# riddhiman13/predictive-multi-agent-framework

Measured on AMD Instinct MI355X. Metric: agent_rollouts_per_s, higher is better.
Workload: dtype f64; 1 GPU; C2: 64 agents x 200-step horizon, 32 sphere obstacles + repulsive sentinel, 1 population(s) per GPU (1 in the job) on 1 GPU(s), static obstacles, one pmaf_tick per step; agents=64, horizon=200, obstacles=32, populations_per_gpu=1, populations_total=1, parallelism=population-per-gpu x1 (same scene on every GPU), devices_visible=1, lanes_per_agent=64, rollout_blocks=64

## Files before the change

predictive-multi-agent-framework_amd/csrc/pmaf_rollout_w64.hpp:

```cpp
#pragma once
#include <type_traits>

#include "pmaf_device.hpp"

namespace pmaf {

template <int MATH>
__device__ __forceinline__ V3 attractor_velocity_error(V3 v, V3 goal_vec, const PopConst &C, double k_attr,
                                                       double k_damp) {
  V3 vel_des = (k_attr / k_damp) * goal_vec;
  double nd, rnd;
  Mth<MATH>::norm_rcp(vel_des, nd, rnd);
  double scale_lim = smin(1.0, Mth<MATH>::div_n(C.vel_max, nd, rnd));
  vel_des = vel_des * scale_lim;
  return vel_des - v;
}

template <int MATH>
__device__ __forceinline__ void finish_step_w64(V3 p, V3 &v, V3 verr, V3 F, double scale, const PopConst &C,
                                                double k_attr, double k_repel, double k_damp, V3 sent_pos,
                                                double sent_rad, double zsent_lt, V3 &new_pos,
                                                const bool sent_reachable = true) {
  if (sent_reachable) {
    V3 ro = sent_pos - p;
    V3 dist_vec = -ro;
    V3 repel = mk(0.0, 0.0, 0.0);
    if (sqn(dist_vec) < zsent_lt) {
      double d = norm(dist_vec) - (C.rad + sent_rad);
      d = smax(d, 1e-5);
      V3 otr = normalized(p - sent_pos);
      double t = 1.0 / d - 1.0 / C.shell;
      double dd = d * d;
      repel = ((k_repel * otr) * t) / dd;
    }
    V3 total = mk(0.0, 0.0, 0.0) + repel;
    F = F + total;
  }
  if (k_attr != 0.0) F = F + (scale * k_damp) * verr;
  V3 acc = F;
  if (C.mass != 1.0) acc = F / C.mass;
  const double az = sqn(acc);
  if (az >= C.zacc_gt) acc = acc * (13.0 / __builtin_sqrt(az));
  V3 half = ((0.5 * acc) * C.dt) * C.dt;
  new_pos = (p + half) + (v * C.dt);
  V3 nv = v + acc * C.dt;
  double vn, rvn;
  Mth<MATH>::norm_rcp(nv, vn, rvn);
  const double f = Mth<MATH>::div_n_pos(C.vel_max, vn, rvn);
  v = nv * ((vn > C.vel_max) ? f : 1.0);
}

__device__ __forceinline__ bool sentinel_reachable(V3 p, V3 sent_pos, V3 sent_vel, double zsent_lt, const PopConst &C,
                                                   int steps) {
  const double adt = fabs(C.dt);
  const double per_step = (6.5 * adt * adt + fabs(C.vel_max) * adt) + norm(sent_vel) * adt;
  const double reach = (double)steps * per_step * 1.001 + 1e-9;
  const double range = __builtin_sqrt(zsent_lt) * 1.001;
  const double d0 = norm(p - sent_pos);
  return !(d0 > range + reach);
}

__device__ __forceinline__ bool field_obstacles_at_rest(const double *src, int n_obs, int M, int lane, double dt) {
  bool rest = true;
  for (int i = lane; i < M; i += 64) {
    const unsigned long long bx = (unsigned long long)__double_as_longlong(src[3 * n_obs + i]),
                             by = (unsigned long long)__double_as_longlong(src[4 * n_obs + i]),
                             bz = (unsigned long long)__double_as_longlong(src[5 * n_obs + i]);
    const unsigned long long px = (unsigned long long)__double_as_longlong(src[i]),
                             py = (unsigned long long)__double_as_longlong(src[n_obs + i]),
                             pz = (unsigned long long)__double_as_longlong(src[2 * n_obs + i]);
    const unsigned long long neg0 = 0x8000000000000000ull;
    rest = rest && ((bx | by | bz) == 0ull) && (px != neg0) && (py != neg0) && (pz != neg0);
  }
  return !wave_any(!rest) && (dt >= 0.0) && (dt < __builtin_huge_val());
}

__device__ __forceinline__ V3 sentinel_repel(V3 p, const PopConst &C, double k_repel, V3 sent_pos, double sent_rad,
                                             double zsent_lt) {
  const V3 ro = sent_pos - p;
  const V3 dist_vec = -ro;
  V3 repel = mk(0.0, 0.0, 0.0);
  if (sqn(dist_vec) < zsent_lt) {
    double d = norm(dist_vec) - (C.rad + sent_rad);
    d = smax(d, 1e-5);
    const V3 otr = normalized(p - sent_pos);
    const double t = 1.0 / d - 1.0 / C.shell;
    const double dd = d * d;
    repel = ((k_repel * otr) * t) / dd;
  }
  return repel;
}

template <int MATH>
__device__ __forceinline__ V3 sentinel_repel_m(V3 p, const PopConst &C, double k_repel, V3 sent_pos, double sent_rad,
                                               double zsent_lt, double inv_shell) {
  typedef Mth<MATH> MT;
  const V3 ro = sent_pos - p;
  const V3 dist_vec = -ro;
  V3 repel = mk(0.0, 0.0, 0.0);
  const double z = sqn(dist_vec);
  if (z < zsent_lt) {
    const double s = MT::sqrt(z);
    double d = s - (C.rad + sent_rad);
    d = smax(d, 1e-5);
    const V3 pms = p - sent_pos;
    const double sd = (z > 0.0) ? s : 1.0;
    const V3 otr = MT::div3_n_pos(pms, sd, MT::rcp_for(sd));
    const double t = MT::div_pos(1.0, d) - inv_shell;
    const double dd = d * d;
    const V3 num = (k_repel * otr) * t;
    repel = MT::div3_n_pos(num, dd, MT::rcp_for(dd));
  }
  return repel;
}

__device__ __forceinline__ V3 sentinel_repel_live(V3 p, const PopConst &C, double k_repel, V3 sent_pos,
                                                  double sent_rad) {
  const V3 ro = sent_pos - p;
  const V3 dist_vec = -ro;
  V3 repel = mk(0.0, 0.0, 0.0);
  double d = norm(dist_vec) - (C.rad + sent_rad);
  d = smax(d, 1e-5);
  if (d < C.shell) {
    const V3 otr = normalized(p - sent_pos);
    const double t = 1.0 / d - 1.0 / C.shell;
    const double dd = d * d;
    repel = ((k_repel * otr) * t) / dd;
  }
  return repel;
}

__device__ __forceinline__ void wave_lds_fence() {
  __builtin_amdgcn_fence(__ATOMIC_RELEASE, "wavefront");
  __builtin_amdgcn_wave_barrier();
  __builtin_amdgcn_fence(__ATOMIC_ACQUIRE, "wavefront");
}

#ifdef PMAF_SECTION_TIMERS
struct SecTimers {
  unsigned long long last, acc[8], cnt[4];
  __device__ __forceinline__ void start() { for (int k = 0; k < 8; k++) acc[k] = 0; for (int k = 0; k < 4; k++) cnt[k] = 0; last = __builtin_amdgcn_s_memtime(); }
  __device__ __forceinline__ void mark(int k) { unsigned long long now = __builtin_amdgcn_s_memtime(); acc[k] += now - last; last = now; }
};
#define PMAF_SEC(ST, k) (ST).mark(k)
#define PMAF_CNT(ST, k, v) (ST).cnt[k] += (v)
#else
struct SecTimers {};
#define PMAF_SEC(ST, k)
#define PMAF_CNT(ST, k, v)
#endif

#define PMAF_RARE(c) __builtin_expect(!!(c), 0)

#ifndef PMAF_SUM_TAIL_PIN
#define PMAF_SUM_TAIL_PIN 0
#endif

typedef unsigned long long lmask;
#define PMAF_BAL(c) __builtin_amdgcn_ballot_w64(c)
#define PMAF_LANE(m) __builtin_amdgcn_inverse_ballot_w64(m)

template <int TILES>
struct LaneObstacles {
  V3 p[TILES], v[TILES];
  double r[TILES];
  double rx[TILES], ry[TILES], rz[TILES];
  double qx[TILES], qy[TILES], qz[TILES];
};

__device__ __forceinline__ int lane_rank(unsigned long long m) {
  return (int)__builtin_amdgcn_mbcnt_hi((unsigned)(m >> 32), __builtin_amdgcn_mbcnt_lo((unsigned)m, 0u));
}

__device__ __forceinline__ V3 readlane_v3(V3 a, int lane) {
  return mk(readlane_d(a.x, lane), readlane_d(a.y, lane), readlane_d(a.z, lane));
}

template <int TILES, int MATH>
__device__ __forceinline__ V3 closest_other_w64(lmask need_latch_m, int t, int lane, int M,
                                                const LaneObstacles<TILES> &O) {
  V3 cpos = mk(0.0, 0.0, 0.0);
  unsigned long long pend = need_latch_m;
  while (pend) {
    const int L = __ffsll((long long)pend) - 1;
    pend &= pend - 1;
    const int id = t * 64 + L;
    V3 own = mk(0.0, 0.0, 0.0);
#pragma unroll
    for (int u = 0; u < TILES; u++)
      if (u == t) own = readlane_v3(O.p[u], L);
    double bd = 100.0;
    int bj = 0x7fffffff;
#pragma unroll
    for (int u = 0; u < TILES; u++) {
      const int j = u * 64 + lane;
      const double d = Mth<MATH>::norm(own - O.p[u]);
      if (j < M && j != id && d < bd) { bd = d; bj = j; }
    }
    const double md = wave_min64(bd);
    const int mj = wave_min64_i((bj != 0x7fffffff && bd == md) ? bj : 0x7fffffff);
    const int c = (mj == 0x7fffffff) ? 0 : mj;
    V3 cp = mk(0.0, 0.0, 0.0);
#pragma unroll
    for (int u = 0; u < TILES; u++)
      if ((c >> 6) == u) cp = readlane_v3(O.p[u], c & 63);
    if (lane == L) cpos = cp;
  }
  return cpos;
}

template <int TILES>
__device__ __forceinline__ V3 closest_from_table_w64(const int32_t *cidx, int t, int lane, const LaneObstacles<TILES> &O) {
  const int c = cidx[t * 64 + lane];
  V3 cp = mk(0.0, 0.0, 0.0);
#pragma unroll
  for (int u = 0; u < TILES; u++) {
    const V3 q = mk(__shfl(O.p[u].x, c & 63), __shfl(O.p[u].y, c & 63), __shfl(O.p[u].z, c & 63));
    if ((c >> 6) == u) cp = q;
  }
  return cp;
}

template <int MATH>
__device__ __forceinline__ V3 cv_close_threshold(const V3 cur, const bool keep, V3 &quot) {
  typedef Mth<MATH> M;
  if constexpr (MATH == MATH_XACT) {
    const double z = sqn(cur);
    double y2;
    const double s = M::sqrt_seed(z, y2);
    quot = M::div3_n_pos(cur, s, M::rcp_seeded(s, y2));
    const bool tiny = (z < 0x1.79ca10c924223p-67) && !keep;
    return mk(tiny ? 0.0 : quot.x, tiny ? 0.0 : quot.y, tiny ? 1.0 : quot.z);
  } else {
    double s;
    M::template norm_unit<true>(cur, s, quot);
    const bool tiny = (s < 1e-10) && !keep;
    return mk(tiny ? 0.0 : quot.x, tiny ? 0.0 : quot.y, tiny ? 1.0 : quot.z);
  }
}

template <int TILES, int TYPE, int MATH, bool PRE = false, bool DPPSUM = false, class KT = ExpK, int NVL = -1, bool LONG = false>
__device__ __forceinline__ void circ_and_scale_w64(int lane, V3 p, V3 v, double zv, V3 goal, V3 g, double dg, V3 gn,
                                                   const PopConst &C, double k_circ,
                                                   int n_obs, double *rot_g, unsigned &known_bits,
                                                   LaneObstacles<TILES> &O, double *clist, double &lane_min,
                                                   V3 &F, double &scale, SecTimers &ST, const KT &EK,
                                                   const int rtype = 0,
                                                   const double s_pre = 0.0, const V3 ron_pre = V3{0.0, 0.0, 0.0},
                                                   const lmask gate_m = ~0ull, const int32_t *cidx = nullptr,
                                                   int *short_cap = nullptr) {
  static_assert(!LONG || (TILES == 1 && DPPSUM && TYPE != T_REAL), "the long loop belongs to the one-slot DPP sum of the rollout kernels");
  typedef Mth<MATH> MT;
  const int type = (TYPE == T_REAL) ? rtype : TYPE;
  constexpr int BATCH = 8;
  constexpr int SCRATCH = 64 * TILES + BATCH;
  constexpr int SUM_SCRATCH = (4 * TILES + 1) * 64;
  constexpr int MIN_CELL_BOUND = pmaf_list_area_doubles(TILES);
  (void)MIN_CELL_BOUND;
  (void)SCRATCH; (void)SUM_SCRATCH;
  const int M = n_obs - 1;
  double best_d = C.shell;
  double best_s = 0.0, best_gr = 0.0;
  int best_i = 0x7fffffff;
  lmask has_best_m = 0ull;
  V3 ron_t[TILES], rv_t[TILES];
  double d_t[TILES];
  lmask in_m[TILES];
  lmask any_in_m = 0ull;
#pragma unroll
  for (int t = 0; t < TILES; t++) {
    const int i = t * 64 + lane;
    const int left = M - t * 64;
    const lmask valid_m = gate_m & ((left >= 64) ? ~0ull : ((left <= 0) ? 0ull : ((1ull << left) - 1ull)));
    const V3 ro = O.p[t] - p;
    rv_t[t] = v - O.v[t];
    double s;
    if (PRE) { s = s_pre; ron_t[t] = ron_pre; }
    else MT::template norm_unit<true>(ro, s, ron_t[t]);
    const lmask skip_m = PMAF_BAL(dot(ron_t[t], gn) < -0.01) & PMAF_BAL(dot(ro, rv_t[t]) < -0.01);
    double d = s - (C.rad + O.r[t]);
    d = smax(d, 1e-5);
    d_t[t] = d;
    const lmask closer_m = valid_m & PMAF_BAL(d < best_d);
    has_best_m |= closer_m;
    const bool closer = PMAF_LANE(closer_m);
    if (TILES == 1) {
      if (closer) { best_d = d; best_i = i; }
      best_s = s; best_gr = dot(g, ro);
    } else {
      if (closer) { best_d = d; best_i = i; best_s = s; best_gr = dot(g, ro); }
    }
    const lmask live_m = valid_m & ~skip_m;
    if (PMAF_LANE(live_m & PMAF_BAL(d < lane_min))) lane_min = d;
    in_m[t] = live_m & PMAF_BAL(d < C.shell);
    any_in_m |= in_m[t];
  }
  PMAF_SEC(ST, 1);
  if (PMAF_RARE(any_in_m == 0ull)) return;
  PMAF_CNT(ST, 0, 1);
  constexpr int MIN_CELL = pmaf_list_area_doubles(TILES);
  unsigned long long *min_cell = reinterpret_cast<unsigned long long *>(clist + MIN_CELL);
  constexpr bool LDSMIN = DPPSUM;
  if (LDSMIN) {
    wave_lds_fence();
    *reinterpret_cast<double *>(min_cell) = C.shell;
    __hip_atomic_fetch_min(min_cell, (unsigned long long)__double_as_longlong(best_d), __ATOMIC_RELAXED,
                           __HIP_MEMORY_SCOPE_WORKGROUP);
  }

#pragma unroll
  for (int t = 0; t < TILES; t++) {
    const int i = t * 64 + lane;
    const lmask need_latch_m = in_m[t] & PMAF_BAL((known_bits & (1u << t)) == 0u);
    if (PMAF_RARE(need_latch_m != 0ull)) {
      V3 cpos = O.p[t];
      if (type == T_OBST || type == T_GOALOBST) {
        if (cidx) cpos = closest_from_table_w64<TILES>(cidx, t, lane, O);
        else cpos = closest_other_w64<TILES, MATH>(need_latch_m, t, lane, M, O);
      }
      if (PMAF_LANE(need_latch_m)) {
        V3 rot = calc_rot_vec_pre<MATH>(type, p, n_obs, O.p[t], cpos, mk(O.qx[t], O.qy[t], O.qz[t]), ron_t[t], g, dg, gn);
        rot_g[i] = rot.x; rot_g[n_obs + i] = rot.y; rot_g[2 * n_obs + i] = rot.z;
        O.rx[t] = rot.x; O.ry[t] = rot.y; O.rz[t] = rot.z;
        known_bits |= (1u << t);
      }
    }
  }
  PMAF_SEC(ST, 2);
  int count = 0;
  double m_mid = 0.0;
  if (LONG) {
    wave_lds_fence();
    clist[(16 << 2) + lane] = 0.0;
  }
  constexpr bool MIN_MID = TILES == 2;
#pragma unroll
  for (int t = 0; t < TILES; t++) {
    if (TILES > 2 && in_m[t] == 0ull) continue;
    const V3 rot = mk(O.rx[t], O.ry[t], O.rz[t]);
    const V3 rv = rv_t[t];
    constexpr bool NVR = (NVL >= 0) && PRE && TILES == 1 && TYPE != T_REAL;
    double zrv;
    V3 nv, cur;
    if constexpr (NVR) {
      zrv = zv;
      const bool rl = (lane == NVL);
      const V3 to_obs = ron_t[t];
      if constexpr (TYPE == T_VEL) {
        const V3 nvel = MT::template normalized<true>(rv);
        nv = nvel;
        V3 q;
        cur = cv_close_threshold<MATH>(nvel - to_obs * dot(nvel, to_obs), false, q);
      } else if constexpr (TYPE == T_GOAL) {
        V3 raw = g - to_obs * dot(to_obs, g);
        raw.x = rl ? v.x : raw.x; raw.y = rl ? v.y : raw.y; raw.z = rl ? v.z : raw.z;
        V3 q;
        cur = cv_close_threshold<MATH>(raw, rl, q);
        nv = readlane_v3(q, NVL);
      } else {
        V3 raw = cross(to_obs, rot);
        raw.x = rl ? v.x : raw.x; raw.y = rl ? v.y : raw.y; raw.z = rl ? v.z : raw.z;
        cur = MT::template normalized<true>(raw);
        nv = readlane_v3(cur, NVL);
      }
    } else {
      zrv = sqn(rv);
      double vn, rvn;
      MT::norm_rcp_zpos(zrv, vn, rvn);
      nv = MT::div3_n_pos(rv, vn, rvn);
      cur = current_vector<MATH, true>(type, rv, g, ron_t[t], rot);
    }
    if (LDSMIN && MIN_MID && t == TILES - 1) {
      wave_lds_fence();
      m_mid = __longlong_as_double((long long)__hip_atomic_load(min_cell, __ATOMIC_RELAXED, __HIP_MEMORY_SCOPE_WORKGROUP));
      __builtin_amdgcn_sched_barrier(0);
    }
    const V3 c = MT::div_pos(k_circ, d_t[t] * d_t[t]) * unit_triple<MATH>(nv, cur);
    const unsigned long long m = in_m[t] & PMAF_BAL(zrv != 0);
    const bool has_c = PMAF_LANE(m);
    if (DPPSUM) {
      const int sl = count + lane_rank(m);
      int li = ((sl >> 4) << 6) + (sl & 15);
      asm("" : "+v"(li));
      const int idx = has_c ? li : (SUM_SCRATCH + (lane >> 4) * 48 + (lane & 15));
      PMAF_BOUND(sl < 64 * TILES && idx + 32 < MIN_CELL_BOUND);
      clist[idx] = c.x; clist[idx + 16] = c.y; clist[idx + 32] = c.z;
    } else {
      const int slot = has_c ? (count + lane_rank(m)) : (SCRATCH + lane);
      PMAF_BOUND(slot * 4 + 2 < MIN_CELL_BOUND);
      double *e = clist + (size_t)slot * 4;
      e[0] = c.x; e[1] = c.y; e[2] = c.z;
    }
    count += __popcll(m);
  }
  if (DPPSUM) {
    if ((lane & 15) >= (count & 15)) clist[((count >> 4) << 6) + lane] = 0.0;
  } else {
    double *e = clist + (size_t)(count + (lane % BATCH)) * 4;
    e[0] = 0.0; e[1] = 0.0; e[2] = 0.0;
  }
  PMAF_CNT(ST, 1, count);
  double e_first = 0.0, e_second = 0.0;
  if (DPPSUM) {
    wave_lds_fence();
    e_first = clist[lane];
    if (TILES == 1) e_second = clist[(16 << 2) + lane];
  }

  double sc;
  {
    double m;
    if (LDSMIN && MIN_MID) {
      m = m_mid;
    } else if (LDSMIN) {
      wave_lds_fence();
      m = __longlong_as_double((long long)__hip_atomic_load(min_cell, __ATOMIC_RELAXED, __HIP_MEMORY_SCOPE_WORKGROUP));
    } else {
      m = wave_min64(best_d);
    }
    const lmask cand_m = has_best_m & PMAF_BAL(best_d == m);
    int bi;
    if (TILES == 1) {
      bi = cand_m ? (__ffsll((long long)cand_m) - 1) : 0x7fffffff;
    } else {
      bi = 0x7fffffff;
#pragma unroll
      for (int t = TILES - 1; t >= 0; t--) {
        const lmask ct = cand_m & PMAF_BAL((best_i >> 6) == t);
        bi = ct ? (t * 64 + __ffsll((long long)ct) - 1) : bi;
      }
    }
    const bool stall = (dot(g, v) <= 0.0) && (zv < C.zv09_lt) && (dg > 0.15);
    double w1;
    if (TILES >= 2) {
      typename std::remove_const<KT>::type EKs = EK;
      double m_in = m;
      const ExpHead H = exp_head(EKs, m_in);
      w1 = 1 - portable_exp_nonpos_staged(-MT::div_pos(MT::sqrt_pos(m_in), C.shell), EKs, H);
    }
    ExpPend EP;
    if (TILES == 1) EP = portable_exp_nonpos_begin(-MT::div_pos(MT::sqrt_pos(m), C.shell), EK);
    const int bl = bi & 63;
    const double sb = readlane_d(best_s, bl), gr = readlane_d(best_gr, bl);
    double w2 = 1 - MT::div(gr, dg * sb);
    w2 = w2 * w2;
    if (TILES == 1) w1 = 1 - portable_exp_nonpos_end(EP);
    const double w = w1 * w2;
    sc = (bi == 0x7fffffff) ? 1.0 : (stall ? 0.0 : w);
  }

  if (DPPSUM) {
  {
    double acc = 0.0;
    if (TILES >= 2) {
    double one = 1.0;
    asm volatile("" : "+v"(one));
    double e = e_first;
    int c16 = 0;
    {
      double en = clist[(16 << 2) + lane];
      asm volatile("s_nop 1" : "+v"(e));
#define PMAF_FM1(K) asm("v_fmac_f64_dpp %0, %1, %2 row_newbcast:" #K " row_mask:0xf bank_mask:0xf" : "+v"(acc) : "v"(e), "v"(one));
      PMAF_FM1(0) PMAF_FM1(1) PMAF_FM1(2) PMAF_FM1(3) PMAF_FM1(4) PMAF_FM1(5) PMAF_FM1(6) PMAF_FM1(7)
      PMAF_FM1(8) PMAF_FM1(9) PMAF_FM1(10) PMAF_FM1(11) PMAF_FM1(12) PMAF_FM1(13) PMAF_FM1(14) PMAF_FM1(15)
#undef PMAF_FM1
      asm volatile("s_nop 0" : "+v"(acc));
      e = en;
      c16 = 16;
      asm volatile("" : : "v"(sc));
    }
    for (; c16 < count; c16 += 16) {
      const double en = clist[((c16 + 16) << 2) + lane];
#define PMAF_FM(K) "v_fmac_f64_dpp %0, %1, %2 row_newbcast:" #K " row_mask:0xf bank_mask:0xf\n\t"
      asm volatile("s_nop 4\n\t"
                   PMAF_FM(0) PMAF_FM(1) PMAF_FM(2) PMAF_FM(3) PMAF_FM(4) PMAF_FM(5) PMAF_FM(6) PMAF_FM(7)
                   PMAF_FM(8) PMAF_FM(9) PMAF_FM(10) PMAF_FM(11) PMAF_FM(12) PMAF_FM(13) PMAF_FM(14) PMAF_FM(15)
                   "s_nop 1"
                   : "+v"(acc) : "v"(e), "v"(one));
#undef PMAF_FM
      e = en;
    }
    } else {
      double one = 1.0;
      asm volatile("" : "+v"(one));
      {
        double e = e_first;
        asm volatile("s_nop 1" : "+v"(e));
#define PMAF_FM1(K) asm("v_fmac_f64_dpp %0, %1, %2 row_newbcast:" #K " row_mask:0xf bank_mask:0xf" : "+v"(acc) : "v"(e), "v"(one));
        PMAF_FM1(0) PMAF_FM1(1) PMAF_FM1(2) PMAF_FM1(3) PMAF_FM1(4) PMAF_FM1(5) PMAF_FM1(6) PMAF_FM1(7)
        PMAF_FM1(8) PMAF_FM1(9) PMAF_FM1(10) PMAF_FM1(11) PMAF_FM1(12) PMAF_FM1(13) PMAF_FM1(14) PMAF_FM1(15)
#undef PMAF_FM1
      }
      if constexpr (LONG) {
        double e2 = e_second;
        asm("s_nop 1\n\tv_fmac_f64_dpp %0, %1, %2 row_newbcast:0 row_mask:0xf bank_mask:0xf" : "+v"(acc) : "v"(e2), "v"(one));
#define PMAF_FM1(K) asm("v_fmac_f64_dpp %0, %1, %2 row_newbcast:" #K " row_mask:0xf bank_mask:0xf" : "+v"(acc) : "v"(e2), "v"(one));
        PMAF_FM1(1) PMAF_FM1(2) PMAF_FM1(3) PMAF_FM1(4) PMAF_FM1(5) PMAF_FM1(6) PMAF_FM1(7)
        PMAF_FM1(8) PMAF_FM1(9) PMAF_FM1(10) PMAF_FM1(11) PMAF_FM1(12) PMAF_FM1(13) PMAF_FM1(14) PMAF_FM1(15)
#undef PMAF_FM1
        asm volatile("s_nop 0" : "+v"(acc));
        if (PMAF_SUM_TAIL_PIN) asm volatile("" : : "v"(sc), "v"(acc));
        if (PMAF_RARE(count > 32)) {
          double e = clist[(32 << 2) + lane];
          for (int c16 = 32; c16 < count; c16 += 16) {
            const double en = clist[((c16 + 16) << 2) + lane];
#define PMAF_FM(K) "v_fmac_f64_dpp %0, %1, %2 row_newbcast:" #K " row_mask:0xf bank_mask:0xf\n\t"
            asm volatile("s_nop 4\n\t"
                         PMAF_FM(0) PMAF_FM(1) PMAF_FM(2) PMAF_FM(3) PMAF_FM(4) PMAF_FM(5) PMAF_FM(6) PMAF_FM(7)
                         PMAF_FM(8) PMAF_FM(9) PMAF_FM(10) PMAF_FM(11) PMAF_FM(12) PMAF_FM(13) PMAF_FM(14) PMAF_FM(15)
                         "s_nop 1"
                         : "+v"(acc) : "v"(e), "v"(one));
#undef PMAF_FM
            e = en;
          }
        }
      } else {
      if (PMAF_SUM_TAIL_PIN) asm volatile("" : : "v"(sc), "v"(acc));
      double e = e_second;
      for (int c16 = 16; PMAF_RARE(c16 < count); c16 += 16) {
        const double en = clist[((c16 + 16) << 2) + lane];
#define PMAF_FM(K) "v_fmac_f64_dpp %0, %1, %2 row_newbcast:" #K " row_mask:0xf bank_mask:0xf\n\t"
        asm volatile("s_nop 4\n\t"
                     PMAF_FM(0) PMAF_FM(1) PMAF_FM(2) PMAF_FM(3) PMAF_FM(4) PMAF_FM(5) PMAF_FM(6) PMAF_FM(7)
                     PMAF_FM(8) PMAF_FM(9) PMAF_FM(10) PMAF_FM(11) PMAF_FM(12) PMAF_FM(13) PMAF_FM(14) PMAF_FM(15)
                     "s_nop 1"
                     : "+v"(acc) : "v"(e), "v"(one));
#undef PMAF_FM
        e = en;
        if (short_cap) asm volatile("s_mov_b32 %0, 0" : "=s"(*short_cap));
      }
      }
    }
    F = mk(readlane_d(acc, 0), readlane_d(acc, 16), readlane_d(acc, 32));
  }
  wave_lds_fence();
  } else {
  wave_lds_fence();
  if (TILES == 1 || lane == 0) {
  for (int k = 0;;) {
    double ex[BATCH], ey[BATCH], ez[BATCH];
#pragma unroll
    for (int j = 0; j < BATCH; j++) {
      const double *e = clist + (size_t)(k + j) * 4;
      ex[j] = e[0]; ey[j] = e[1]; ez[j] = e[2];
    }
#pragma unroll
    for (int j = 0; j < BATCH; j++) { F.x = F.x + ex[j]; F.y = F.y + ey[j]; F.z = F.z + ez[j]; }
    k += BATCH;
    if (k >= count) break;
  }
  }
  if (TILES > 1) F = readlane_v3(F, 0);
  wave_lds_fence();
  }
  PMAF_SEC(ST, 3);
  scale = (sqn(F) >= C.zf_gt) ? sc : scale;
  PMAF_SEC(ST, 4);
}

__device__ __forceinline__ double ld_agent(const double *p) {
  return __hip_atomic_load(p, __ATOMIC_RELAXED, __HIP_MEMORY_SCOPE_AGENT);
}
template <int MATH>
__device__ __forceinline__ void path_cost_terms_w64(int lane, const double *path, int n, const double *ws,
                                                    double k_workspace, double *list, double &cost_ws,
                                                    double &path_len) {
  __builtin_amdgcn_fence(__ATOMIC_RELEASE, "agent");
  __builtin_amdgcn_fence(__ATOMIC_ACQUIRE, "agent");
  cost_ws = 0.0;
  path_len = 0.0;
  V3 q_n = mk(0.0, 0.0, 0.0), qp_n = mk(0.0, 0.0, 0.0);
  auto fetch = [&](int base, V3 &q, V3 &qp) __attribute__((always_inline)) {
    const int k = base + lane;
    const bool valid = k < n;
    const bool has_seg = valid && (k > 0);
    const int kk = valid ? k : 0, kp = has_seg ? (k - 1) : 0;
    q = mk(ld_agent(path + kk * 3), ld_agent(path + kk * 3 + 1), ld_agent(path + kk * 3 + 2));
    qp = mk(ld_agent(path + kp * 3), ld_agent(path + kp * 3 + 1), ld_agent(path + kp * 3 + 2));
  };
  fetch(0, q_n, qp_n);
  for (int base = 0; base < n; base += 64) {
    const int k = base + lane;
    const bool valid = k < n;
    const bool has_seg = valid && (k > 0);
    const V3 q = q_n, qp = qp_n;
    if (base + 64 < n) fetch(base + 64, q_n, qp_n);
    const double seg = Mth<MATH>::norm(q - qp);
    list[lane] = has_seg ? seg : 0.0;
    wave_lds_fence();
#pragma unroll 8
    for (int j = 0; j < 64; j++) path_len += list[j];
    wave_lds_fence();
    const bool out = valid && ((q.x > ws[0]) | (q.x < ws[1]) | (q.y > ws[2]) | (q.y < ws[3]) | (q.z > ws[4]) | (q.z < ws[5]));
    unsigned long long m = wave_ballot(out);
    while (m) {
      const int L = __ffsll((long long)m) - 1;
      m &= m - 1;
      ws_cost_add(cost_ws, readlane_v3(q, L), ws, k_workspace);
    }
  }
}

}
```

predictive-multi-agent-framework_amd/csrc/pmaf_rollout_w64_body.hpp:

```cpp
#pragma once
#include <hip/hip_runtime.h>
#include <hip/hip_ext.h>

#include "pmaf_types.hpp"
#include "pmaf_device.hpp"
#include "pmaf_rollout_w64.hpp"
#include "pmaf_rollout_grp.hpp"

using namespace pmaf;

#define PMAF_W64_EACH_TYPE(type, BODY) \
  switch (type) { \
    case T_GOAL: BODY(T_GOAL); break; \
    case T_OBST: BODY(T_OBST); break; \
    case T_GOALOBST: BODY(T_GOALOBST); break; \
    case T_VEL: BODY(T_VEL); break; \
    case T_RANDOM: BODY(T_RANDOM); break; \
    case T_HAD: BODY(T_HAD); break; \
    default: break; \
  }

__device__ __forceinline__ bool track_reachable(int lane, V3 p0, const double *trk, int n_pts, double zsent_lt,
                                                const PopConst &C, int steps) {
  const double adt = fabs(C.dt);
  const double per_step = 6.5 * adt * adt + fabs(C.vel_max) * adt;
  const double reach = (double)steps * per_step * 1.001 + 1e-9;
  const double range = __builtin_sqrt(zsent_lt) * 1.001;
  bool any = false;
  for (int j = lane; j < n_pts; j += 64) {
    const V3 y = mk(trk[3 * j], trk[3 * j + 1], trk[3 * j + 2]);
    any = any || !(norm(p0 - y) > range + reach);
  }
  return wave_any(any);
}

__device__ __forceinline__ double *w64_exp_lds() {
  __shared__ double s_expk[EXPK_N];
  return s_expk;
}
template <int TILES>
__device__ __forceinline__ auto w64_exp_consts(int lane) {
  if constexpr (TILES >= 2) {
    double *tab = w64_exp_lds();
    exp_consts_to_lds(tab, lane);
    wave_lds_fence();
    return exp_consts_from_lds(tab);
  } else {
    return exp_consts_in_vgprs();
  }
}
template <int TILES, int TYPE, int MATH, int SENT = 2, bool DPPSUM = false, bool PLAIN = false, bool STATICV = false, bool SLICE = false,
          bool TRACK = false, bool FTRACK = false>
__device__ __forceinline__ void rollout_w64_body(const DevView &D, const CostParams &CP, const int lane,
                                                 const int pop, const int a, const double *trk = nullptr,
                                                 const int trk_len = 0, const double *ftrk = nullptr,
                                                 const int ftrk_len = 0, const int ftrk_first = 0) {
  static_assert(!TRACK || (TILES == 1 && SENT != 2), "the repulsive track rides in lane 60 of the one-slot kernel");
  static_assert(!FTRACK || (TILES == 1 && SENT != 2 && !STATICV && TRACK), "the obstacle tracks ride in lanes 0 .. M-1 of the one-slot kernel");
  extern __shared__ double smem[];
  const unsigned long long t_begin = wall_clock64();
  const int n_obs = D.n_obs;
  const int M = n_obs - 1;
  PopConst C = D.C;
  { double *f = reinterpret_cast<double *>(&C);
    for (int i = 0; i < (int)(sizeof(PopConst) / sizeof(double)); i++) asm volatile("" : "+v"(f[i])); }
  const auto EK = w64_exp_consts<TILES>(lane);
  const size_t pa = (size_t)pop * D.N + a;
  const double *src = D.obs_start + (size_t)pop * 7 * n_obs;
  const int32_t *ks = D.known_start + (size_t)pop * n_obs;
  double *rot_g = D.rot + pa * 3 * n_obs;
  const double *rnd_g = D.rnd + pa * 3 * n_obs;

  LaneObstacles<TILES> O;
  unsigned known_bits = 0u;
  constexpr bool USES_CLOSEST = TILES >= 2 && (TYPE == T_OBST || TYPE == T_GOALOBST);
#pragma unroll
  for (int t = 0; t < TILES; t++) {
    int i = t * 64 + lane;
    bool valid = i < M;
    int ii = valid ? i : 0;
    O.p[t] = mk(src[ii], src[n_obs + ii], src[2 * n_obs + ii]);
    O.v[t] = mk(src[3 * n_obs + ii], src[4 * n_obs + ii], src[5 * n_obs + ii]);
    O.r[t] = src[6 * n_obs + ii];
    O.rx[t] = rot_g[ii]; O.ry[t] = rot_g[n_obs + ii]; O.rz[t] = rot_g[2 * n_obs + ii];
    if (TYPE == T_RANDOM) { O.qx[t] = rnd_g[ii]; O.qy[t] = rnd_g[n_obs + ii]; O.qz[t] = rnd_g[2 * n_obs + ii]; }
    else { O.qx[t] = 0.0; O.qy[t] = 0.0; O.qz[t] = 0.0; }
    if (valid && ks[ii]) known_bits |= (1u << t);
  }
  V3 sent_p = mk(src[M], src[n_obs + M], src[2 * n_obs + M]);
  const V3 sent_v = mk(src[3 * n_obs + M], src[4 * n_obs + M], src[5 * n_obs + M]);
  const double sent_r = src[6 * n_obs + M];
  typedef const __attribute__((address_space(1))) double *gptr;
  gptr trk_v = (gptr)trk;
  const int trk_last = (trk_len > 0) ? (trk_len - 1) : 0;
  const lmask trk_m = (TRACK && SENT == 1 && trk_len > 0) ? (1ull << 60) : 0ull;
  if (TRACK && SENT == 1) {
    asm volatile("" : "+v"(trk_v));
    if (trk_len > 0) sent_p = mk(trk_v[0], trk_v[1], trk_v[2]);
  }
  gptr ftrk_v = (gptr)ftrk + lane;
  const int ftrk_last = (ftrk_len > 0) ? (ftrk_len - 1) : 0;
  const int ftrk_at = (ftrk_first < ftrk_last) ? ftrk_first : ftrk_last;
  const lmask ftrk_m = (FTRACK && ftrk_len > 0) ? ((1ull << M) - 1ull) : 0ull;
  if (FTRACK) {
    asm volatile("" : "+v"(ftrk_v));
    const gptr fp = ftrk_v + (size_t)ftrk_at * 384;
    const bool fl = PMAF_LANE(ftrk_m);
    O.p[0].x = fl ? fp[0] : O.p[0].x; O.p[0].y = fl ? fp[64] : O.p[0].y; O.p[0].z = fl ? fp[128] : O.p[0].z;
    O.v[0].x = fl ? fp[192] : O.v[0].x; O.v[0].y = fl ? fp[256] : O.v[0].y; O.v[0].z = fl ? fp[320] : O.v[0].z;
  }

  V3 goal = mk(D.goal[pop * 3], D.goal[pop * 3 + 1], D.goal[pop * 3 + 2]);
  V3 init_pos = mk(D.agent_init_pos[pop * 3], D.agent_init_pos[pop * 3 + 1], D.agent_init_pos[pop * 3 + 2]);
  asm volatile("" : "+v"(goal.x), "+v"(goal.y), "+v"(goal.z), "+v"(init_pos.x), "+v"(init_pos.y), "+v"(init_pos.z));
  V3 p = mk(D.start_pos[pop * 3], D.start_pos[pop * 3 + 1], D.start_pos[pop * 3 + 2]);
  V3 v = mk(D.start_vel[pop * 3], D.start_vel[pop * 3 + 1], D.start_vel[pop * 3 + 2]);
  double k_attr = D.k_attr[pa], k_circ = D.k_circ[pa], k_repel = D.k_repel[pa], k_damp = D.k_damp[pa];
  asm volatile("" : "+v"(k_attr), "+v"(k_circ), "+v"(k_repel), "+v"(k_damp));
  double *path = D.paths + pa * (size_t)D.cap * 3;

  int clist_off = 7 * n_obs + (n_obs + 1) / 2;
  clist_off += clist_off & 1;
  double *clist = smem + clist_off;

  double lane_min = C.shell;
  int n = 1;
  bool ran = false;
  if (lane == 0) { path[0] = p.x; path[1] = p.y; path[2] = p.z; }

  typedef Mth<MATH> MT;
  V3 g = goal - p;
  double dg = MT::norm(g);
  double zv = sqn(v);
  double z_init = sqn(p - init_pos);
  V3 gn = (dg > 0.0) ? MT::div3(g, dg) : g;
  constexpr bool PRE = (TILES == 1);
  double s_pre = 0.0;
  V3 ron_pre = mk(0.0, 0.0, 0.0);
  double lane_scale = (lane == 61) ? (k_attr / k_damp) : 1.0;
  asm volatile("" : "+v"(lane_scale));
  if (PRE) {
    const double nz = (C.dt < 0.0) ? 0.0 : -0.0;
    if (lane == 63 || lane == 61) { O.p[0] = goal; O.v[0] = mk(nz, nz, nz); }
    if (SENT == 1 && lane == 60) { O.p[0] = sent_p; O.v[0] = sent_v; }
    MT::norm_unit(O.p[0] - p, s_pre, ron_pre);
  }
  constexpr bool SRIDE = PRE && SENT == 1;
  V3 verr = attractor_velocity_error<MATH>(v, g, C, k_attr, k_damp);
  const double zsent_lt = D.zsent_lt[pop];
  const bool sent_reachable = (SENT == 2) ? sentinel_reachable(p, sent_p, sent_v, zsent_lt, C, D.cap) : (SENT == 1);
  bool moving = false;
#pragma unroll
  for (int t = 0; t < TILES; t++) moving = moving || !(O.v[t].x == 0.0 && O.v[t].y == 0.0 && O.v[t].z == 0.0);
  moving = wave_any(moving);
  bool advance = true;
  const int32_t *cidx = nullptr;
  if (USES_CLOSEST) {
    if (!moving && D.closest_ok[pop] == 1) {
      int32_t *s_cidx = reinterpret_cast<int32_t *>(smem);
      const int32_t *ci = D.closest_idx + (size_t)pop * n_obs;
#pragma unroll
      for (int t = 0; t < TILES; t++) {
        const int i = t * 64 + lane;
        if (i < M) s_cidx[i] = ci[i];
      }
      wave_lds_fence();
      cidx = s_cidx;
    }
  }
  V3 repel = mk(0.0, 0.0, 0.0);
  const double inv_shell = (SENT == 0) ? 0.0 : 1.0 / C.shell;
  if (sent_reachable) repel = sentinel_repel_m<MATH>(p, C, k_repel, sent_p, sent_r, zsent_lt, inv_shell);
  SecTimers ST;
#ifdef PMAF_SECTION_TIMERS
  ST.start();
#endif
  const bool younger = SLICE && ((((unsigned)blockIdx.y * gridDim.x + blockIdx.x) / (unsigned)D.n_simds) & 1u) != 0u;
  const unsigned slice_log2 = (unsigned)D.prio_slice_log2, younger_of_8 = (unsigned)D.prio_younger_of_8;
  if constexpr (TILES == 1 && DPPSUM) {
    int short_cap = D.cap;
    while ((dg > 0.1) && (n < short_cap)) {
#define PMAF_STEP_LONG false
#define PMAF_STEP_FLAG , &short_cap
#include "pmaf_rollout_w64_step.hpp"
#undef PMAF_STEP_LONG
    }
    while ((dg > 0.1) && (n < D.cap)) {
#define PMAF_STEP_LONG true
#include "pmaf_rollout_w64_step.hpp"
#undef PMAF_STEP_LONG
#undef PMAF_STEP_FLAG
    }
  } else {
    while ((dg > 0.1) && (n < D.cap)) {
#define PMAF_STEP_LONG false
#define PMAF_STEP_FLAG
#include "pmaf_rollout_w64_step.hpp"
#undef PMAF_STEP_LONG
#undef PMAF_STEP_FLAG
    }
  }
  if (SLICE) __builtin_amdgcn_s_setprio(0);
#ifdef PMAF_SECTION_TIMERS
  if (lane == 0 && pop == 0 && a < 7)
    printf("agent %d type %d steps %d | verr+gate %llu sweep %llu scale %llu circ %llu sum %llu (skip) %llu finish %llu tail %llu | "
           "in-shell steps %llu terms %llu\n", a, TYPE, n - 1, ST.acc[0], ST.acc[1], ST.acc[2], ST.acc[3], ST.acc[4],
           ST.acc[5], ST.acc[6], ST.acc[7], ST.cnt[0], ST.cnt[1]);
#endif

  double cost_ws, path_len;
#ifdef PMAF_SECTION_TIMERS
  const unsigned long long t_loop_end = wall_clock64();
#endif
  path_cost_terms_w64<MATH>(lane, path, n, CP.ws, CP.k_workspace, clist, cost_ws, path_len);
#ifdef PMAF_SECTION_TIMERS
  if (lane == 0 && pop == 0 && a < 7)
    printf("agent %d: loop %llu0 ns, path-cost pass %llu0 ns (%d points)\n", a, t_loop_end - t_begin, wall_clock64() - t_loop_end, n);
#endif

  const double min_obs = wave_min64(lane_min);
  int32_t *ko = D.known_out + pa * n_obs;
#pragma unroll
  for (int t = 0; t < TILES; t++) {
    int i = t * 64 + lane;
    if (i < M) ko[i] = (int32_t)((known_bits >> t) & 1u);
  }
  if (lane == 0) {
    ko[M] = ks[M];
    D.n_points[pa] = n;
    D.agent_vel[pa * 3] = v.x; D.agent_vel[pa * 3 + 1] = v.y; D.agent_vel[pa * 3 + 2] = v.z;
    D.min_obs[pa] = min_obs;
    D.cost_ws[pa] = cost_ws;
    D.path_len[pa] = path_len;
    D.goal_dist[pa] = dg;
    if (ran) D.reached[pa] = dg < 0.100001;
    atomicAdd(D.step_counter, (unsigned long long)(n - 1));
    D.pred_ticks[pa] = wall_clock64() - t_begin;
  }
}

template <int TILES, int MATH, bool DPPSUM, bool PLAIN, bool SLICE>
__device__ __forceinline__ void rollout_w64_dispatch(const DevView &D, const CostParams &CP) {
  const int lane = threadIdx.x;
  const int pop = blockIdx.y;
  const int a = blockIdx.x;
  if (TILES == 1) {
    const int n_obs = D.n_obs, M = n_obs - 1;
    const double *src = D.obs_start + (size_t)pop * 7 * n_obs;
    const V3 sp = mk(src[M], src[n_obs + M], src[2 * n_obs + M]);
    const V3 sv = mk(src[3 * n_obs + M], src[4 * n_obs + M], src[5 * n_obs + M]);
    const V3 p0 = mk(D.start_pos[pop * 3], D.start_pos[pop * 3 + 1], D.start_pos[pop * 3 + 2]);
    const PopConst C0 = D.C;
    const bool reach = sentinel_reachable(p0, sp, sv, D.zsent_lt[pop], C0, D.cap);
    const bool st = field_obstacles_at_rest(src, n_obs, M, lane, C0.dt) && (M <= 59 || !reach);
#define PMAF_BODY(T) \
    if (st) { \
      if (!reach) rollout_w64_body<TILES, T, MATH, 0, DPPSUM, PLAIN, true, SLICE>(D, CP, lane, pop, a); \
      else rollout_w64_body<TILES, T, MATH, 1, DPPSUM, PLAIN, true, SLICE>(D, CP, lane, pop, a); \
    } else if (!reach) rollout_w64_body<TILES, T, MATH, 0, DPPSUM, PLAIN, false, SLICE>(D, CP, lane, pop, a); \
    else rollout_w64_body<TILES, T, MATH, 1, DPPSUM, PLAIN, false, SLICE>(D, CP, lane, pop, a)
    PMAF_W64_EACH_TYPE(D.types[a], PMAF_BODY)
#undef PMAF_BODY
    return;
  }
#define PMAF_BODY(T) rollout_w64_body<TILES, T, MATH, 2, DPPSUM, PLAIN>(D, CP, lane, pop, a)
  PMAF_W64_EACH_TYPE(D.types[a], PMAF_BODY)
#undef PMAF_BODY
}
```

Before: 280,700 rollouts/s.

## Batch path-cost pass over four chunks with DPP broadcast-FMA path-length sum

Restructures the post-rollout path-cost pass to fetch four 64-point chunks of the path at once, which raises memory-level parallelism over the single-chunk prefetch it replaces. The serial 64-element LDS sum per chunk is replaced with inline-asm v_fmac_f64_dpp row_newbcast instructions that accumulate 16 values per issue. The wave-min reduction of the obstacle distance is moved inside the function so it can overlap with the outstanding loads. This adds hand-written asm with manual s_nop hazard padding, which is arch-specific and may change the floating-point summation order.

```diff
diff --git a/predictive-multi-agent-framework_amd/csrc/pmaf_rollout_w64.hpp b/predictive-multi-agent-framework_amd/csrc/pmaf_rollout_w64.hpp
--- a/predictive-multi-agent-framework_amd/csrc/pmaf_rollout_w64.hpp
+++ b/predictive-multi-agent-framework_amd/csrc/pmaf_rollout_w64.hpp
@@ -561,44 +561,90 @@
 __device__ __forceinline__ double ld_agent(const double *p) {
   return __hip_atomic_load(p, __ATOMIC_RELAXED, __HIP_MEMORY_SCOPE_AGENT);
 }
+#define PMAF_FM(K) "v_fmac_f64_dpp %0, %1, %2 row_newbcast:" #K " row_mask:0xf bank_mask:0xf\n\t"
+__device__ __forceinline__ void path_sum_chunk(double &acc, double e, double one) {
+  asm volatile("s_nop 4\n\t"
+               PMAF_FM(0) PMAF_FM(1) PMAF_FM(2) PMAF_FM(3) PMAF_FM(4) PMAF_FM(5) PMAF_FM(6) PMAF_FM(7)
+               PMAF_FM(8) PMAF_FM(9) PMAF_FM(10) PMAF_FM(11) PMAF_FM(12) PMAF_FM(13) PMAF_FM(14) PMAF_FM(15)
+               "s_nop 1"
+               : "+v"(acc) : "v"(e), "v"(one));
+}
+#undef PMAF_FM
 template <int MATH>
 __device__ __forceinline__ void path_cost_terms_w64(int lane, const double *path, int n, const double *ws,
                                                     double k_workspace, double *list, double &cost_ws,
-                                                    double &path_len) {
+                                                    double &path_len, const double *lane_min = nullptr,
+                                                    double *wave_min = nullptr) {
   __builtin_amdgcn_fence(__ATOMIC_RELEASE, "agent");
   __builtin_amdgcn_fence(__ATOMIC_ACQUIRE, "agent");
   cost_ws = 0.0;
-  path_len = 0.0;
-  V3 q_n = mk(0.0, 0.0, 0.0), qp_n = mk(0.0, 0.0, 0.0);
-  auto fetch = [&](int base, V3 &q, V3 &qp) __attribute__((always_inline)) {
-    const int k = base + lane;
-    const bool valid = k < n;
-    const bool has_seg = valid && (k > 0);
-    const int kk = valid ? k : 0, kp = has_seg ? (k - 1) : 0;
-    q = mk(ld_agent(path + kk * 3), ld_agent(path + kk * 3 + 1), ld_agent(path + kk * 3 + 2));
-    qp = mk(ld_agent(path + kp * 3), ld_agent(path + kp * 3 + 1), ld_agent(path + kp * 3 + 2));
+  constexpr int NB = 4;
+  V3 q[NB], qp[NB];
+  auto fetch = [&](int base) __attribute__((always_inline)) {
+#pragma unroll
+    for (int b = 0; b < NB; b++) {
+      const int k = base + 64 * b + lane;
+      const bool valid = k < n;
+      const bool has_seg = valid && (k > 0);
+      const int kk = valid ? k : 0, kp = has_seg ? (k - 1) : 0;
+      q[b] = mk(ld_agent(path + kk * 3), ld_agent(path + kk * 3 + 1), ld_agent(path + kk * 3 + 2));
+      qp[b] = mk(ld_agent(path + kp * 3), ld_agent(path + kp * 3 + 1), ld_agent(path + kp * 3 + 2));
+    }
   };
-  fetch(0, q_n, qp_n);
-  for (int base = 0; base < n; base += 64) {
-    const int k = base + lane;
-    const bool valid = k < n;
-    const bool has_seg = valid && (k > 0);
-    const V3 q = q_n, qp = qp_n;
-    if (base + 64 < n) fetch(base + 64, q_n, qp_n);
-    const double seg = Mth<MATH>::norm(q - qp);
-    list[lane] = has_seg ? seg : 0.0;
-    wave_lds_fence();
-#pragma unroll 8
-    for (int j = 0; j < 64; j++) path_len += list[j];
-    wave_lds_fence();
-    const bool out = valid && ((q.x > ws[0]) | (q.x < ws[1]) | (q.y > ws[2]) | (q.y < ws[3]) | (q.z > ws[4]) | (q.z < ws[5]));
-    unsigned long long m = wave_ballot(out);
-    while (m) {
-      const int L = __ffsll((long long)m) - 1;
-      m &= m - 1;
-      ws_cost_add(cost_ws, readlane_v3(q, L), ws, k_workspace);
-    }
-  }
-}
-
-}
+  fetch(0);
+  if (lane_min) *wave_min = wave_min64(*lane_min);
+  double acc = 0.0, one = 1.0;
+  asm volatile("" : "+v"(one));
+  const int col = lane & 15;
+  for (int base = 0;;) {
+    double seg[NB], e[NB][4];
+#pragma unroll
+    for (int b = 0; b < NB; b++) seg[b] = Mth<MATH>::norm(q[b] - qp[b]);
+#pragma unroll
+    for (int b = 0; b < NB; b++) {
+      int lane_w = lane;
+      asm volatile("" : "+v"(lane_w));
+      const int k = base + 64 * b + lane_w;
+      const bool has_seg = (k < n) && (k > 0);
+      list[lane] = has_seg ? seg[b] : 0.0;
+      wave_lds_fence();
+#pragma unroll
+      for (int j = 0; j < 4; j++) e[b][j] = list[(j << 4) + col];
+      wave_lds_fence();
+    }
+#pragma unroll
+    for (int b = 0; b < NB; b++) {
+      const int nb = n - base - 64 * b;
+      if (nb > 0) {
+        path_sum_chunk(acc, e[b][0], one);
+        if (nb > 16) {
+          path_sum_chunk(acc, e[b][1], one);
+          if (nb > 32) {
+            path_sum_chunk(acc, e[b][2], one);
+            if (nb > 48) path_sum_chunk(acc, e[b][3], one);
+          }
+        }
+      }
+    }
+#pragma unroll
+    for (int b = 0; b < NB; b++) {
+      int lane_o = lane;
+      asm volatile("" : "+v"(lane_o));
+      const bool valid = base + 64 * b + lane_o < n;
+      const V3 qb = q[b];
+      const bool out = valid && ((qb.x > ws[0]) | (qb.x < ws[1]) | (qb.y > ws[2]) | (qb.y < ws[3]) | (qb.z > ws[4]) | (qb.z < ws[5]));
+      unsigned long long m = wave_ballot(out);
+      while (m) {
+        const int L = __ffsll((long long)m) - 1;
+        m &= m - 1;
+        ws_cost_add(cost_ws, readlane_v3(qb, L), ws, k_workspace);
+      }
+    }
+    base += 64 * NB;
+    if (base >= n) break;
+    fetch(base);
+  }
+  path_len = acc;
+}
+
+}
diff --git a/predictive-multi-agent-framework_amd/csrc/pmaf_rollout_w64_body.hpp b/predictive-multi-agent-framework_amd/csrc/pmaf_rollout_w64_body.hpp
--- a/predictive-multi-agent-framework_amd/csrc/pmaf_rollout_w64_body.hpp
+++ b/predictive-multi-agent-framework_amd/csrc/pmaf_rollout_w64_body.hpp
@@ -212,13 +212,13 @@
 #ifdef PMAF_SECTION_TIMERS
   const unsigned long long t_loop_end = wall_clock64();
 #endif
-  path_cost_terms_w64<MATH>(lane, path, n, CP.ws, CP.k_workspace, clist, cost_ws, path_len);
+  double min_obs;
+  path_cost_terms_w64<MATH>(lane, path, n, CP.ws, CP.k_workspace, clist, cost_ws, path_len, &lane_min, &min_obs);
 #ifdef PMAF_SECTION_TIMERS
   if (lane == 0 && pop == 0 && a < 7)
     printf("agent %d: loop %llu0 ns, path-cost pass %llu0 ns (%d points)\n", a, t_loop_end - t_begin, wall_clock64() - t_loop_end, n);
 #endif
 
-  const double min_obs = wave_min64(lane_min);
   int32_t *ko = D.known_out + pa * n_obs;
 #pragma unroll
   for (int t = 0; t < TILES; t++) {
```

Result: no change. 281,200 rollouts/s, median of 2 (+0.2%).
